# JuliaControl/ModelPredictiveControl.jl

Hardware: AMD Instinct MI355X
Metric: QP solves/sec (moveinput!) (higher is better)
Workload: dtype f64

## Files before the change

### modelpredictivecontrol.jl_amd/csrc/mpcqp_bodies.h

```cpp
#pragma once
#include <math.h>

#include <type_traits>

#include "mpcqp_types.h"

#if defined(MPCQP_PROFILE) && defined(__HIP_DEVICE_COMPILE__)
#define MPCQP_TIC() const long long tic_ = clock64()
#define MPCQP_TOC(i) prof_[i] += (double)(clock64() - tic_)
#define MPCQP_TICK(name) const long long name = clock64()
#define MPCQP_TOCK(i, name) prof_[i] += (double)(clock64() - name)
#elif defined(MPCQP_ISA_MARKERS) && defined(__HIP_DEVICE_COMPILE__)
#define MPCQP_MARK_(txt) do { __builtin_amdgcn_sched_barrier(0); asm volatile("; MPCQP_MARK " txt ::: "memory"); __builtin_amdgcn_sched_barrier(0); } while (0)
#define MPCQP_TIC() MPCQP_MARK_("tic")
#define MPCQP_TOC(i) MPCQP_MARK_("toc " #i)
#define MPCQP_TICK(name) MPCQP_MARK_("tic " #name)
#define MPCQP_TOCK(i, name) MPCQP_MARK_("toc " #i)
#define MPCQP_MTIC() MPCQP_MARK_("tic")
#define MPCQP_MTOC(name) MPCQP_MARK_("toc " name)
#else
#define MPCQP_TIC() ((void)0)
#define MPCQP_TOC(i) ((void)0)
#define MPCQP_TICK(name) ((void)0)
#define MPCQP_TOCK(i, name) ((void)0)
// ... 152 lines not shown
    }
    static bool matches(const Dims& d) { return matches_dims(d) && d.gmask == GMASK; }
};

template <class DM>
constexpr bool has_w() {
    if constexpr (DM::is_static) return DM::nw > 0;
    else return true;
}

constexpr int NROWARR = 7;

struct Carve {
    int S, Phi, zero, z, dz, q, zlo, zhi, gt, rd, dinv, zb, xh, F, tA[NPAIR], tB[NPAIR], ucum, exT, Wm;
    int rows[NROWARR];
    int jl, blk;
    int total;
};

template <class DM>
MPCQP_HD constexpr bool one_row_per_lane() {
    if constexpr (DM::is_static) return DM::nZ <= WAVE;
    else return false;
}

template <class DM>
MPCQP_HD constexpr int hwq_() {
    if constexpr (DM::is_static) {
        constexpr int n = (DM::nY + WAVE - 1) / WAVE;
        return (DM::nZ <= WAVE && n <= 4) ? n : 0;
    } else {
        return 0;
    }
}

template <class DM>
MPCQP_HD inline int stride_S(const DM& d) {
    if constexpr (DM::is_static) return DM::sp;
    else return d.ny * d.nu;
}

template <class DM>
MPCQP_HD inline int zpad_S(const DM&) {
    if constexpr (DM::is_static) return DM::zpad;
    else return 0;
}
// ... 515 lines not shown
                acc1 += ok ? p1 : 0.0;
            }
            if constexpr (REG) mine_k += scale * (acc0 + acc1);
            else out[k] += scale * (acc0 + acc1);
        }
    }

    MPCQP_HD static void unpack_idx(int idx, int& i, int& ip) {
        i = (int)((sqrt(8.0 * idx + 1.0) - 1.0) * 0.5);
        while (i * (i + 1) / 2 > idx) --i;
        while ((i + 1) * (i + 2) / 2 <= idx) ++i;
        ip = idx - i * (i + 1) / 2;
    }

#if defined(__HIP_DEVICE_COMPILE__)
    typedef double v4d __attribute__((ext_vector_type(4)));
    template <int I0, int NT, class F>
    static __device__ __forceinline__ void etde_passes(F& f) {
        if constexpr (I0 < NT) {
            f(std::integral_constant<int, I0>{});
            etde_passes<(I0 == 0 ? 2 : I0 + 1), NT>(f);
        }
    }
    __device__ __forceinline__ int EtDE_add_mfma(const double* dd, double* P, double scale, const double* tb,
                                                 const double* Hg = nullptr, bool ow = false) {
        if constexpr (W::NTEAM > 1) { static_assert(W::WV == 0, MPCQP_POST_WV0); w.post(TJ_ETDE, (int)(dd - sm), (int)(P - sm), tb ? (int)(tb - sm) : 0, (ow ? 1 : 0) | (Hg ? 2 : 0) | (tb ? 4 : 0), scale); }
        const int e = EtDE_share(dd, P, scale, tb ? tb : dd, Hg, ow, tb != nullptr);
        if constexpr (W::NTEAM > 1) w.join();
        return e;
    }
    __device__ __forceinline__ int EtDE_share(const double* dd, double* P, double scale, const double* tb, const double* Hg, bool ow, bool has_tb) {
        return EtDE_share_(dd, P, scale, tb, Hg, ow, has_tb);
    }
    __device__ __forceinline__ int EtDE_share_(const double* dd, double* P, double scale, const double* tb, const double* Hg, bool ow, bool has_tb) {
        ow = ow || Hg != nullptr;
        constexpr int NU = DM::nu, NY = DM::ny, NDU = DM::nDU, NYR = DM::nY, SP = DM::sp, RS = DM::rs;
        constexpr int NT = (NDU + 15) / 16, NK = (NYR + 3) / 4;
        const int li = w.lane & 15, lk = w.lane >> 4;
        const int lkp = (NY % 4 == 0) ? (((lk & 1) << 1) | (lk >> 1)) : lk;
        int offI[NT], offL[NT], jI[NT];
        MPCQP_UNROLL
        for (int I = 0; I < NT; ++I) {
            const int i = 16 * I + li;
            const int j = i / NU, cc = i - j * NU;
            const int tj = jl(i < NDU ? j : 0);
            jI[I] = i < NDU ? tj : (1 << 20);
            offI[I] = -tj * SP + cc;
            offL[I] = offI[I] + lkp * RS;
        }
        constexpr int IE = NDU / 16, LE = NDU % 16;
        int eps_t0 = -1;
        if (DM::neps && has_tb && IE < NT) {
            int v = (jl((16 * IE) / NU) * NY) / 4;
            v = v < NK ? v : NK;
            if ((4 * v) % NY != 0) v = 0;
            eps_t0 = (4 * v) / NY;
        }
// ... 10 lines not shown
        }
        auto pass = [&](auto I0c) {
            constexpr int I0 = decltype(I0c)::value;
            if constexpr (W::NTEAM > 1) {
                if constexpr (!team_mine_mfma<W>(I0 == 0 ? 0 : I0 - 1)) return;
            }
            constexpr int MAXT = NT + 1;
            constexpr int I1 = (I0 == 0 && NT > 1) ? 1 : I0;
            v4d acc[2][MAXT];
            MPCQP_UNROLL
            for (int x = 0; x < 2; ++x) {
                MPCQP_UNROLL
                for (int J = 0; J < MAXT; ++J) acc[x][J] = v4d{0.0, 0.0, 0.0, 0.0};
            }
            const bool erow = DM::neps && has_tb && IE >= I0 && IE <= I1;
            auto entry_ok = [&](int I, int J, int reg) {
                const bool eI = erow && I == IE;
                const int il = 4 * reg + lk;
                const bool rowok = 16 * I + 15 < NDU || 16 * I + il < NDU;
                const bool colok = 16 * J + 15 < NDU || 16 * J + li < NDU;
                const bool low = J < I || li <= il;
                return colok && ((rowok && low) || (eI && il == LE));
            };
            auto entry_idx = [&](int I, int J, int reg) {
                const int G = 4 * I + reg;
                return 8 * G * (G + 1) + 16 * J + 4 * (G + 1) * lk + li;
            };
            double hreg[2][MAXT][4];
            auto hload = [&]() {
                MPCQP_UNROLL
                for (int I = I0; I <= I1; ++I) {
                    MPCQP_UNROLL
                    for (int J = 0; J <= I; ++J) {
                        MPCQP_UNROLL
                        for (int reg = 0; reg < 4; ++reg)
                            hreg[I - I0][J][reg] = Hg[entry_ok(I, J, reg) ? (unsigned)entry_idx(I, J, reg) : 0u];
                    }
                }
            };
            constexpr bool LATEH = !VREG && NT > 4;
            if (Hg && !VREG && !LATEH) hload();
            auto kfirst = [&](int I) {
                int v = (jl((16 * I) / NU) * NY) / 4;
                v = v < NK ? v : NK;
                if (erow && I == IE) { if ((4 * v) % NY != 0) v = 0; }
                return v;
            };
            const int kB = (I1 > I0) ? kfirst(I1) : NK;
            const int kA = kfirst(I0) < kB ? kfirst(I0) : kB;
            const int zoff = (int)((sm + c.zero) - S);
            struct Ops { double dv, tbv, e[NT]; };
            auto kload = [&](int kk, Ops& o) {
                o.tbv = 0.0;
                if constexpr (NY % 4 == 0) {
                    const int t = (4 * kk) / NY, a0 = 4 * kk - t * NY;
                    const int base = t * SP + a0 * RS;
                    o.dv = dd[4 * kk + lkp];
                    if (erow) o.tbv = tb[4 * kk + lkp];
                    MPCQP_UNROLL
// ... 71 lines not shown
            for (int kk = kA; kk < kB1; ++kk) {
                if (PIPE) { kload(kk + 1, nxt); MPCQP_SCHED_FENCE(); kcomp(cur, true, false); MPCQP_SCHED_FENCE(); cur = nxt; }
                else { kload(kk, cur); kcomp(cur, true, false); }
            }
            if (LATEH && I1 == I0) {
                if (Hg) hload();
                MPCQP_SCHED_FENCE();
                MPCQP_PRAGMA(unroll MPCQP_ETDE_UNROLL)
                for (int kk = kB1; kk < kB; ++kk) {
                    if (PIPE) { kload(kk + 1, nxt); MPCQP_SCHED_FENCE(); kcomp(cur, true, false); MPCQP_SCHED_FENCE(); cur = nxt; }
                    else { kload(kk, cur); kcomp(cur, true, false); }
                }
            }
            if (I1 > I0) {
                if (LATEH && Hg) hload();
                MPCQP_PRAGMA(unroll MPCQP_ETDE_UNROLL)
                for (int kk = kB; kk < NK; ++kk) {
                    if (PIPE) { kload(kk + 1, nxt); MPCQP_SCHED_FENCE(); kcomp(cur, true, true); MPCQP_SCHED_FENCE(); cur = nxt; }
                    else { kload(kk, cur); kcomp(cur, true, true); }
                }
            }
            }
            if (Hg && VREG) hload();
            if (ow) {
                MPCQP_UNROLL
                for (int I = I0; I <= I1; ++I) {
                    MPCQP_UNROLL
                    for (int J = 0; J <= I; ++J) {
                        MPCQP_UNROLL
                        for (int reg = 0; reg < 4; ++reg)
                            if (entry_ok(I, J, reg))
                                P[entry_idx(I, J, reg)] = Hg ? fma(scale, acc[I - I0][J][reg], hreg[I - I0][J][reg]) : scale * acc[I - I0][J][reg];
                    }
                }
                return;
            }
            double* const trash = sm + c.zero + 4;
            MPCQP_UNROLL
            for (int I = I0; I <= I1; ++I) {
                MPCQP_UNROLL
                for (int J = 0; J <= I; ++J) {
                    double* pp_[4];
                    double old_[4];
                    MPCQP_UNROLL
                    for (int reg = 0; reg < 4; ++reg) {
                        pp_[reg] = entry_ok(I, J, reg) ? P + entry_idx(I, J, reg) : trash;
                        old_[reg] = *pp_[reg];
                    }
                    MPCQP_UNROLL
                    for (int reg = 0; reg < 4; ++reg) *pp_[reg] = fma(scale, acc[I - I0][J][reg], old_[reg]);
                }
            }
        };
        etde_passes<0, NT>(pass);
        if constexpr (DM::neps != 0 && W::WV == 0) {
            if (ow && !Hg) {
                if constexpr (IE >= NT) {
                    for (int k = w.lane; k < NDU; k += WAVE) P[pk(NDU, k)] = 0.0;
                }
                if (w.lane == 0) P[pk(NDU, NDU)] = 0.0;
            } else if (Hg) {
                if constexpr (IE >= NT) {
                    for (int k = w.lane; k < NDU; k += WAVE) P[pk(NDU, k)] = Hg[pk(NDU, k)];
                }
                if (w.lane == 0) P[pk(NDU, NDU)] = Hg[pk(NDU, NDU)];
            }
        }
        return eps_t0;
    }
#endif

    MPCQP_HD int EtDE_add(const double* dd, double* P, double scale = 1.0, const double* tb = nullptr,
                          const double* Hg = nullptr, bool ow = false) {
#if defined(__HIP_DEVICE_COMPILE__)
        if constexpr (DM::is_static) return EtDE_add_mfma(dd, P, scale, tb, Hg, ow);
#endif
        const int ny = d.ny, nu = d.nu, nDU = d.nDU;
        const int nstrip = pk_size(nDU) / 4;
        for (int st = w.lane; st < nstrip; st += WAVE) {
            int g = (int)((sqrt(1.0 + 2.0 * st) - 1.0) * 0.5);
            while (2 * g * (g + 1) > st) --g;
            while (2 * (g + 1) * (g + 2) <= st) ++g;
            const int rem = st - 2 * g * (g + 1);
            const int i = 4 * g + rem / (g + 1), ip0 = 4 * (rem % (g + 1));
            if (i >= nDU) continue;
            const int j = i / nu, cc = i - j * nu, t0 = jl(j);
            const double* S2[4];
            MPCQP_UNROLL
            for (int u = 0; u < 4; ++u) {
                const int ip = ip0 + u <= i ? ip0 + u : i;
                const int j2 = ip / nu, c2 = ip - j2 * nu;
                S2[u] = S + (t0 - jl(j2)) * sp + c2;
            }
            const double* S1 = S + cc;
            const double* dt = dd + t0 * ny;
            double acc[4] = {0.0, 0.0, 0.0, 0.0};
            for (int t = t0; t < d.Hp; ++t) {
                for (int a = 0; a < ny; ++a) {
// ... 433 lines not shown
    RowStore<DM> rows;
    double *z, *dz, *q, *zlo, *zhi, *gt, *rd, *F, *Phi;
    int mact;
    double wsum;
    double nh;
    double delta;
    double prof_[16] = {0};
    double myinvd = 0.0;
    double myd_ = 0.0;
    bool chol_broke = false;
    bool fold_H = false;
    bool h_Lnz = false;
    double h2n_ = 0.0, h2l_ = 0.0;
    static constexpr int HWQ = hwq_<DM>();
    double hwy_[HWQ > 0 ? HWQ : 1] = {0.0};
    MPCQP_HD static constexpr bool hwy_cached() { return hwq_<DM>() > 0; }
    MPCQP_HD double hwy(int k) const {
        double v = hwy_[0];
        MPCQP_UNROLL
        for (int q_ = 1; q_ < HWQ; ++q_) v = (k >= WAVE * q_) ? hwy_[q_] : v;
        return v;
    }

    MPCQP_HD Step(Qp<W, DM>& qp_)
        : qp(qp_), w(qp_.w), d(qp_.d), m(qp_.m), b(qp_.b), sm(qp_.sm), c(qp_.c),
          rows(qp_.d, qp_.sm, qp_.c, qp_.w.lane) {
        z = sm + c.z; dz = sm + c.dz; q = sm + c.q; zlo = sm + c.zlo; zhi = sm + c.zhi;
        gt = sm + c.gt; rd = sm + c.rd; F = sm + c.F;
        Phi = qp.Phi;
        delta = d.dual_reg;
    }

    MPCQP_HD double stepc_at(int a, int k) const { return m.stepc[((size_t)b * SC_N + a) * d.nDU + k]; }

    MPCQP_HD double soft_init(int g, int k) const {
        if (!d.neps) return 0.0;
        const double* p = nullptr;
        double def = 0.0;
        switch (g) {
            case 2 * P_U: p = m.C_umin; break;
            case 2 * P_U + 1: p = m.C_umax; break;
            case 2 * P_DU: p = m.C_dumin; break;
            case 2 * P_DU + 1: p = m.C_dumax; break;
            case 2 * P_Y: p = m.C_ymin; def = 1.0; break;
            case 2 * P_Y + 1: p = m.C_ymax; def = 1.0; break;
            case 2 * P_X: p = m.c_x0min; def = 1.0; break;
// ... 596 lines not shown
        qp.Et_apply_add(tY, rd, 2.0);
        double suf = 0.0;
        if (h_Lnz && d.nDU <= WAVE) {
            const double pre = qp.block_prefix(w.lane < d.nDU ? z[w.lane] : 0.0);
            suf = qp.block_suffix(w.lane < d.nDU ? H2L(w.lane) * pre : 0.0);
        }
        for (int k = w.lane; k < d.nZ; k += WAVE) {
            const double hn = one_row_per_lane<DM>() ? h2n_ : H2N_load(k);
            rd[k] = (k < d.nDU ? rd[k] + suf : 0.0) + hn * z[k];
        }
        w.sync();
        MPCQP_TOC(2);
    }

    MPCQP_HD void load_H() {
        if constexpr (W::NTEAM > 1) { static_assert(W::WV == 0, MPCQP_POST_WV0); w.post(TJ_LOADH); }
        load_H_share();
        if constexpr (W::NTEAM > 1) w.join();
        w.sync();
    }
    MPCQP_HD void load_H_share() {
        const double* H = m.Hpk + (size_t)b * d.npk;
        constexpr int NB = 8;
        const int n = d.npk, stride = WAVE * W::NTEAM;
        for (int i0 = WAVE * W::WV; i0 < n; i0 += NB * stride) {
            double v[NB];
            MPCQP_UNROLL
            for (int q_ = 0; q_ < NB; ++q_) { const int i = i0 + w.lane + stride * q_; v[q_] = H[i < n ? i : 0]; }
            MPCQP_UNROLL
            for (int q_ = 0; q_ < NB; ++q_) { const int i = i0 + w.lane + stride * q_; if (i < n) Phi[i] = v[q_]; }
        }
    }

    MPCQP_HD bool phi_direct() const {
#if defined(__HIP_DEVICE_COMPILE__)
        return fold_H || (DM::is_static && qp.pair_on(P_Y));
#else
        return fold_H;
#endif
    }
    MPCQP_HD bool etde_overwrites() const {
#if defined(__HIP_DEVICE_COMPILE__)
        return DM::is_static && qp.pair_on(P_Y);
#else
        return false;
#endif
    }

    MPCQP_HD void GtDG_urows_share() {
        const int nu = d.nu, nDU = d.nDU;
        const double* tU = sm + c.tA[P_U];
        for (int k = w.lane + WAVE * ((W::WV + W::NTEAM - 1) % W::NTEAM); k < nDU; k += WAVE * W::NTEAM) {
            const int j = k / nu, cc = k - j * nu;
            const double suf = tU[k];
            MPCQP_PRAGMA(unroll MPCQP_URMW_UNROLL)
            for (int j2 = 0; j2 <= j; ++j2) Phi[pk(k, j2 * nu + cc)] += suf;
        }
    }
    MPCQP_HD void GtDG_xrows_share() {
        const int nDU = d.nDU, ntri = nDU * (nDU + 1) / 2;
        const double* tX = sm + c.tA[P_X];
        for (int idx = w.lane + WAVE * W::WV; idx < ntri; idx += WAVE * W::NTEAM) {
            int i, ip;
            Qp<W, DM>::unpack_idx(idx, i, ip);
            double acc = 0.0;
            for (int r = 0; r < d.nxh; ++r) acc += qp.Xat(r, i) * tX[r] * qp.Xat(r, ip);
            Phi[pk(i, ip)] += acc;
        }
    }
    MPCQP_HD void GtDG_wrows_share() {
        if constexpr (has_w<DM>()) {
            const int nu = d.nu, nDU = d.nDU, ntri = nDU * (nDU + 1) / 2, nw = d.nw;
            const double* dW = sm + c.tA[P_W];
            for (int idx = w.lane + WAVE * W::WV; idx < ntri; idx += WAVE * W::NTEAM) {
                int i, ip;
                Qp<W, DM>::unpack_idx(idx, i, ip);
                const int j = i / nu, cc = i - j * nu, j2 = ip / nu, c2 = ip - j2 * nu;
                double acc = 0.0;
                for (int t = 0; t <= d.Hp; ++t)
                    for (int iw = 0; iw < nw; ++iw) {
                        const double dk = dW[t * nw + iw];
                        if (dk != 0.0) acc += dk * qp.Ew_at(t, iw, j, cc) * qp.Ew_at(t, iw, j2, c2);
                    }
                Phi[pk(i, ip)] += acc;
            }
        }
    }

    template <class Fn>
    MPCQP_HD void add_GtDG(Fn dd) {
        MPCQP_TIC();
        const int nu = d.nu, nDU = d.nDU, nZ = d.nZ;
        double ee = 0.0;
        for_pairs([&](int p, int k, Row* r0, Row* r1) {
            double dmin = 0.0, dmax = 0.0, cmin = 0.0, cmax = 0.0;
            if (r0 && fin(*r0)) { dmin = dd(*r0); cmin = r0->cs; }
            if (r1 && fin(*r1)) { dmax = dd(*r1); cmax = r1->cs; }
            double hw = 0.0;
            if (fold_H) {
                if (p == P_Y) hw = hwy_cached() ? hwy(k) : (k < d.nY ? 2.0 * m.Mdiag[(size_t)b * d.nY + k] : 0.0);
                else if (p == P_U) hw = H2L(k);
            }
            sm[c.tA[p] + k] = dmin + dmax + hw;
            if (p != P_BOX) {
                sm[c.tB[p] + k] = cmin * dmin - cmax * dmax;
                ee += cmin * cmin * dmin + cmax * cmax * dmax;
            }
        });
        ee = w.sum(ee);
        w.sync();
        if (fold_H && !etde_overwrites()) {
            for (int i = w.lane; i < d.npk; i += WAVE) Phi[i] = 0.0;
            w.sync();
        }
        bool epsY = qp.pair_on(P_Y), epsU = qp.pair_on(P_U);
        if constexpr (has_w<DM>()) {
            if (qp.pair_on(P_W) && d.neps) {
                qp.W_fold(sm + c.tB[P_W], sm + c.tB[P_Y], !epsY, sm + c.tB[P_U], !epsU);
                epsY = epsU = true;
            }
        }
        MPCQP_TOC(3);
        int eps_t0 = -1;
        if (qp.pair_on(P_Y)) {
            MPCQP_TIC();
            eps_t0 = qp.EtDE_add(sm + c.tA[P_Y], Phi, 1.0, d.neps ? sm + c.tB[P_Y] : nullptr,
                                 (phi_direct() && !fold_H) ? m.Hpk + (size_t)b * d.npk : nullptr, fold_H && etde_overwrites());
            w.sync();
            MPCQP_TOC(4);
        }
        MPCQP_TICK(tic5_);
        if (qp.pair_on(P_U) && nDU <= WAVE) {
            const double* tU = sm + c.tA[P_U];
            const int k = w.lane < nDU ? w.lane : 0;
            const int j = k / nu, cc = k - j * nu;
            const double suf = qp.block_suffix(w.lane < nDU ? tU[k] : 0.0);
            double* const trash = sm + c.zero + 4;
            double* const row = Phi + pk(k, cc);
            if constexpr (DM::is_static) {
                double* q_[DM::Hc];
                double old_[DM::Hc];
                MPCQP_UNROLL
                for (int j2 = 0; j2 < DM::Hc; ++j2) {
                    q_[j2] = (j2 <= j && w.lane < nDU) ? row + j2 * nu : trash;
                    old_[j2] = *q_[j2];
                }
                MPCQP_UNROLL
                for (int j2 = 0; j2 < DM::Hc; ++j2) *q_[j2] = old_[j2] + suf;
            } else {
                for (int j2 = 0; j2 < d.Hc; ++j2) {
                    double* const q_ = (j2 <= j && w.lane < nDU) ? row + j2 * nu : trash;
                    *q_ += suf;
                }
            }
        } else if (qp.pair_on(P_U)) {
            double* tU = sm + c.tA[P_U];
            w.sync();
            block_scan(tU, tU, true);
            if constexpr (W::NTEAM > 1) { static_assert(W::WV == 0, MPCQP_POST_WV0); w.post(TJ_UROWS); }
            GtDG_urows_share();
            if constexpr (W::NTEAM > 1) w.join();
        }
        if (qp.pair_on(P_X)) {
            w.sync();
            if constexpr (W::NTEAM > 1) { static_assert(W::WV == 0, MPCQP_POST_WV0); w.post(TJ_XROWS); }
            GtDG_xrows_share();
            if constexpr (W::NTEAM > 1) w.join();
        }
        if constexpr (has_w<DM>()) {
            if (qp.pair_on(P_W)) {
                w.sync();
                if constexpr (W::NTEAM > 1) { static_assert(W::WV == 0, MPCQP_POST_WV0); w.post(TJ_WROWS); }
                GtDG_wrows_share();
                if constexpr (W::NTEAM > 1) w.join();
            }
        }
        w.sync();
        for (int k = w.lane; k < nZ; k += WAVE) {
            double acc = 0.0;
            if (qp.pair_on(P_BOX)) acc += sm[c.tA[P_BOX] + k];
            if (k < nDU && qp.pair_on(P_DU)) acc += sm[c.tA[P_DU] + k];
            if (k == nZ - 1 && d.neps) acc += ee;
            if (fold_H) acc += one_row_per_lane<DM>() ? h2n_ : H2N_load(k);
            Phi[pk(k, k)] += acc;
        }
        if (d.neps) {
            double* st = dz;
            double sufB = 0.0;
            if (epsU && nDU <= WAVE) sufB = qp.block_suffix(w.lane < nDU ? sm[c.tB[P_U] + w.lane] : 0.0);
            for (int k = w.lane; k < nDU; k += WAVE) {
                double acc = 0.0;
                if (qp.pair_on(P_DU)) acc += sm[c.tB[P_DU] + k];
                if (epsU && nDU <= WAVE) acc += sufB;
                else if (epsU) {
                    const int j = k / nu, cc = k - j * nu;
                    const double* tU = sm + c.tB[P_U];
                    MPCQP_UNROLL4
                    for (int jj = j; jj < d.Hc; ++jj) acc += tU[jj * nu + cc];
                }
                if (qp.pair_on(P_X)) {
                    const double* tX = sm + c.tB[P_X];
                    for (int i = 0; i < d.nxh; ++i) acc += qp.Xat(i, k) * tX[i];
                }
                st[k] = acc;
            }
            if (epsY && eps_t0 != 0) qp.Et_apply_add(sm + c.tB[P_Y], st, 1.0, eps_t0);
            for (int k = w.lane; k < nDU; k += WAVE) Phi[pk(nZ - 1, k)] += st[k];
        }
        w.sync();
        MPCQP_TOCK(5, tic5_);
    }

    MPCQP_HD static long long clock64_() {
#if defined(MPCQP_PROFILE) && defined(__HIP_DEVICE_COMPILE__)
        return clock64();
#else
        return 0;
#endif
    }

    MPCQP_HD static void load4(const double* p, double* x) {
#if defined(__HIP_DEVICE_COMPILE__)
        typedef double v2d_ __attribute__((ext_vector_type(2)));
        const v2d_ a = reinterpret_cast<const v2d_*>(p)[0], b2 = reinterpret_cast<const v2d_*>(p)[1];
        x[0] = a.x; x[1] = a.y; x[2] = b2.x; x[3] = b2.y;
#else
        x[0] = p[0]; x[1] = p[1]; x[2] = p[2]; x[3] = p[3];
#endif
    }
    MPCQP_HD static void store4(double* p, const double* x) {
// ... 5 lines not shown
        p[0] = x[0]; p[1] = x[1]; p[2] = x[2]; p[3] = x[3];
#endif
    }

#if defined(__HIP_DEVICE_COMPILE__)
    template <int P>
    __device__ __forceinline__ void chol_panel_update() {
        if constexpr (W::NTEAM > 1) { static_assert(W::WV == 0, MPCQP_POST_WV0); w.post(TJ_PANEL, P); }
        chol_panel_share<P>();
        if constexpr (W::NTEAM > 1) w.join();
    }
    template <int P>
    __device__ __forceinline__ void chol_panel_share() {
        typedef double v4d_ __attribute__((ext_vector_type(4)));
        constexpr int n = DM::nZ, NT = (n + 15) / 16;
        if constexpr (P < NT) {
            const int li = w.lane & 15, lk = w.lane >> 4;
            auto mine = [](int I) { return team_mine_mfma<W>(I - P); };
            const double* X[NT];
            v4d_ acc[NT];
            MPCQP_UNROLL
            for (int I = P; I < NT; ++I) {
                const int row = 16 * I + li < n ? 16 * I + li : n - 1;
                X[I] = Phi + pk(row, 0) + lk;
                acc[I] = v4d_{0.0, 0.0, 0.0, 0.0};
            }
            if constexpr (team_any_mfma<W>(NT - P)) {
            MPCQP_PRAGMA(unroll MPCQP_PANEL_UNROLL)
            for (int kk = 0; kk < 4 * P; ++kk) {
                const double bb = X[P][4 * kk];
                const double bs = one_row_per_lane<DM>() ? bb * gt[4 * kk + lk] : bb;
                if (mine(P)) acc[P] = __builtin_amdgcn_mfma_f64_16x16x4f64(bb, bs, acc[P], 0, 0, 0);
                MPCQP_UNROLL
                for (int I = P + 1; I < NT; ++I)
                    if (mine(I)) acc[I] = __builtin_amdgcn_mfma_f64_16x16x4f64(X[I][4 * kk], bs, acc[I], 0, 0, 0);
            }
            }
            double* const trash = sm + c.zero + 4;
            MPCQP_UNROLL
            for (int I = P; I < NT; ++I) {
                if (!mine(I)) continue;
                double* pp_[4];
                double old_[4];
                MPCQP_UNROLL
                for (int reg = 0; reg < 4; ++reg) {
                    const int row = 16 * I + lk + 4 * reg, col = 16 * P + li;
                    pp_[reg] = (row < n && col <= row) ? Phi + pk(row, col) : trash;
                    old_[reg] = *pp_[reg];
                }
                MPCQP_UNROLL
                for (int reg = 0; reg < 4; ++reg) *pp_[reg] = old_[reg] - acc[I][reg];
            }
            w.sync();
        }
    }
#endif

#if defined(__HIP_DEVICE_COMPILE__)
    template <int P>
    __device__ __forceinline__ void panel_dispatch(int p) {
        if constexpr (P < (DM::nZ + 15) / 16) {
            if (p == P) chol_panel_share<P>();
            else panel_dispatch<P + 1>(p);
        }
    }
#endif

#if defined(__HIP_DEVICE_COMPILE__)
    template <int P, int Bk>
    __device__ __forceinline__ void chol_block_update() {
        typedef double v4d_ __attribute__((ext_vector_type(4)));
        constexpr int n = DM::nZ, NT = (n + 15) / 16, K0 = 16 * P + 4 * Bk;
        const int li = w.lane & 15, lk = w.lane >> 4;
        double x[NT];
        MPCQP_UNROLL
        for (int T = P; T < NT; ++T) {
            const int row = 16 * T + li < n ? 16 * T + li : n - 1;
            x[T] = Phi[pk(row, 0) + K0 + lk];
        }
        const double xPs = one_row_per_lane<DM>() ? x[P] * gt[K0 + lk] : x[P];
        double* const trash = sm + c.zero + 4;
        double* q_[NT][4];
        double old_[NT][4];
        MPCQP_UNROLL
        for (int T = P; T < NT; ++T) {
            MPCQP_UNROLL
            for (int r = Bk + 1; r < 4; ++r) {
                if (16 * P + 4 * r >= n) continue;
                const int row = 16 * T + li, col = 16 * P + 4 * r + lk;
                q_[T][r] = (row < n && col <= row) ? Phi + pk(row, col) : trash;
                old_[T][r] = *q_[T][r];
            }
        }
        MPCQP_UNROLL
        for (int T = P; T < NT; ++T) {
            const v4d_ acc = __builtin_amdgcn_mfma_f64_16x16x4f64(xPs, x[T], v4d_{0.0, 0.0, 0.0, 0.0}, 0, 0, 0);
            MPCQP_UNROLL
            for (int r = Bk + 1; r < 4; ++r) {
                if (16 * P + 4 * r >= n) continue;
                *q_[T][r] = old_[T][r] - acc[r];
            }
        }
        w.sync();
    }

    template <int K0>
    __device__ __forceinline__ void chol_static(double thr) {
        constexpr int n = DM::nZ, CB = 4, P = K0 / 16, Bk = (K0 % 16) / 4;
        const int i = w.lane;
        const bool act = i < n;
        const int rowi = pk(act ? i : 0, 0);
        if constexpr (Bk == 0 && P > 0) chol_panel_update<P>();
        const bool mine = act && i >= K0;
        double v[CB], lk[CB];
        load4(mine ? Phi + rowi + K0 : sm + c.zero, v);
        constexpr int NCL = (n - K0 < CB) ? n - K0 : CB;
        MPCQP_UNROLL
        for (int cc = 0; cc < CB; ++cc) {
            if (cc < NCL) {
                const int k = K0 + cc;
                const double nidb = -w.bcast(rcp(v[cc]), k);
                lk[cc] = v[cc] * nidb;
                MPCQP_UNROLL
                for (int c2 = cc + 1; c2 < NCL; ++c2) v[c2] = fma(v[cc], w.bcast(lk[cc], K0 + c2), v[c2]);
            } else {
                lk[cc] = 0.0;
            }
        }
        if (mine) {
            const double t0 = (i & 1) ? v[1] : v[0], t1 = (i & 1) ? v[3] : v[2];
            myd_ = (i & 2) ? t1 : t0;
            gt[i] = myd_;
            MPCQP_UNROLL
            for (int cc = 0; cc < CB; ++cc) lk[cc] = (i > K0 + cc) ? lk[cc] : 0.0;
            store4(Phi + rowi + K0, lk);
        }
        w.sync();
        if constexpr (K0 + CB < n) {
            if constexpr (Bk < 3) chol_block_update<P, Bk>();
            chol_static<K0 + CB>(thr);
        }
    }
#endif

    MPCQP_HD void cholesky() {
        if (d.nZ > WAVE) { cholesky_big(); return; }
        cholesky_();
    }
    MPCQP_HD void cholesky_() {
        MPCQP_TIC();
        const int n = d.nZ;
        const int i = w.lane;
        const bool act = i < n;
        const int rowi = pk(act ? i : 0, 0);
        const double dia = act ? Phi[rowi + i] : 1.0;
        const double thr = 1e-14 * fabs(dia);
        const double* zero4 = sm + c.zero;
        myinvd = 0.0;
        constexpr int CB = 4;
#if defined(__HIP_DEVICE_COMPILE__)
        if constexpr (one_row_per_lane<DM>()) {
            chol_static<0>(thr);
            chol_broke = w.any(act && !(myd_ > thr));
            myinvd = act ? rcp(myd_) : 0.0;
            w.sync();
            MPCQP_TOC(6);
            return;
        }
#endif
        MPCQP_NOUNROLL
        for (int k0 = 0; k0 < n; k0 += CB) {
            const bool mine = act && i >= k0;
            double v[CB];
            load4(mine ? Phi + rowi + k0 : zero4, v);
            if (mine && k0 > 0) {
                const double* Li = Phi + rowi;
                const int rb = pk(k0, 0), rs = k0 + CB;
                const double* Lk[CB];
// ... 27 lines not shown
            }
            w.sync();
        }
        myinvd = fmx(myinvd, 1e-32);
        chol_broke = w.any(act && myinvd <= 1e-32);
        MPCQP_TOC(6);
    }

    MPCQP_HD static double rsqrt_(double x) {
#if defined(__HIP_DEVICE_COMPILE__)
        const double r = __builtin_amdgcn_rsq(x);
        return r * fma(-0.5 * x * r, r, 1.5);
#else
        return 1.0 / sqrt(x);
#endif
    }

#if defined(__HIP_DEVICE_COMPILE__)
    template <int T>
    __device__ __forceinline__ void solve_fwd_load(double (*cf)[4], const int rowi, const bool act) {
        constexpr int n = DM::nZ, K0 = 16 * T, KT = (n - K0 < 16) ? n - K0 : 16, NC = (KT + 3) / 4;
        const int i = w.lane;
        MPCQP_UNROLL
        for (int u = 0; u < NC; ++u) load4((act && i >= K0 + 4 * u) ? Phi + rowi + K0 + 4 * u : sm + c.zero, cf[u]);
    }
    template <int T>
    __device__ __forceinline__ void solve_bwd_load(double (*cb)[4]) {
        constexpr int n = DM::nZ, K0 = 16 * T, KT = (n - K0 < 16) ? n - K0 : 16, NC = (KT + 3) / 4;
        const int i = w.lane;
        MPCQP_UNROLL
        for (int u = 0; u < NC; ++u) {
            const int k0 = K0 + 4 * u;
            const double* p = solve_zero_region() ? ((i < k0 + 4 && i < n) ? Phi + pk(k0, 0) + i : sm + c.S)
                                                  : Phi + pk(k0, 0) + (i < k0 + 4 ? i : 0);
            MPCQP_UNROLL
            for (int e = 0; e < 4; ++e) cb[u][e] = (k0 + e < n) ? p[e * (k0 + 4)] : 0.0;
        }
    }
    template <int T>
    __device__ __forceinline__ void solve_fwd_tile(double& r, double (*cf)[4], const int rowi, const bool act) {
        constexpr int n = DM::nZ, NT = (n + 15) / 16, K0 = 16 * T, KT = (n - K0 < 16) ? n - K0 : 16, NC = (KT + 3) / 4;
        double nx[4][4];
        if constexpr (T + 1 < NT) solve_fwd_load<T + 1>(nx, rowi, act);
        else solve_bwd_load<NT - 1>(nx);
        MPCQP_SCHED_FENCE();
        MPCQP_UNROLL
        for (int u = 0; u < NC; ++u) chain_sw<1 << T, false>(u, r, cf[u]);
        if constexpr (T + 1 < NT) {
            const double y = w.fetch(r, K0 + (w.lane & 15));
            double a0 = 0.0, a1 = 0.0;
            MPCQP_UNROLL
            for (int u = 0; u < NC; ++u) rows_sw<0xf & ~((2 << T) - 1)>(u, (u & 1) ? a1 : a0, y, cf[u]);
            r += a0 + a1;
            MPCQP_SCHED_FENCE();
            solve_fwd_tile<T + 1>(r, nx, rowi, act);
// ... 26 lines not shown
            for (int u = 0; u < NC; ++u) rows_sw<(1 << T) - 1>(u, (u & 1) ? a1 : a0, x, cb[u]);
            r += a0 + a1;
            solve_bwd_tile<T - 1>(r, nx, act);
        }
    }
    template <int ROWS, bool REV>
    __device__ __forceinline__ void chain_sw(int u, double& r, const double* cc) {
        switch (u) {
            case 0: W::template chain4<0, ROWS, REV>(r, cc[0], cc[1], cc[2], cc[3]); break;
            case 1: W::template chain4<4, ROWS, REV>(r, cc[0], cc[1], cc[2], cc[3]); break;
            case 2: W::template chain4<8, ROWS, REV>(r, cc[0], cc[1], cc[2], cc[3]); break;
            default: W::template chain4<12, ROWS, REV>(r, cc[0], cc[1], cc[2], cc[3]); break;
        }
    }
    template <int ROWS>
    __device__ __forceinline__ void rows_sw(int u, double& a, double x, const double* cc) {
        switch (u) {
            case 0: W::template fmabc4<0, ROWS>(a, x, cc[0], cc[1], cc[2], cc[3]); break;
            case 1: W::template fmabc4<4, ROWS>(a, x, cc[0], cc[1], cc[2], cc[3]); break;
            case 2: W::template fmabc4<8, ROWS>(a, x, cc[0], cc[1], cc[2], cc[3]); break;
            default: W::template fmabc4<12, ROWS>(a, x, cc[0], cc[1], cc[2], cc[3]); break;
        }
    }
    static constexpr bool solve_zero_region() { return DM::zpad * DM::sp >= 3 * (DM::nZ + 3) + 4; }
    __device__ __forceinline__ void solve_static() {
        const int i = w.lane;
        solve_static_reg(i < DM::nZ ? gt[i] : 0.0);
    }
    __device__ __forceinline__ double solve_static_reg(double r) {
        constexpr int n = DM::nZ;
        const int i = w.lane;
        const bool act = i < n;
        const int rowi = pk(act ? i : 0, 0);
        double cf[4][4];
        solve_fwd_load<0>(cf, rowi, act);
        solve_fwd_tile<0>(r, cf, rowi, act);
        if (act) dz[i] = r;
        w.sync();
        return act ? r : 0.0;
    }
#endif

    MPCQP_HD void solve_into_dz() {
        w.relane();
        if (d.nZ > WAVE) { solve_big(); return; }
        MPCQP_TIC();
#if defined(__HIP_DEVICE_COMPILE__)
        if constexpr (one_row_per_lane<DM>()) {
            solve_static();
            MPCQP_TOC(7);
            return;
        }
#endif
        const int n = d.nZ;
        const int i = w.lane;
        const bool act = i < n;
// ... 406 lines not shown
            int j = 0;
            MPCQP_PRAGMA(unroll MPCQP_HZ_UNROLL)
            for (; j + 1 <= k; j += 2) { h0 += Hk[j] * z[j]; h1 += Hk[j + 1] * z[j + 1]; }
            if (j <= k) h0 += Hk[j] * z[j];
            MPCQP_PRAGMA(unroll MPCQP_HZ_UNROLL)
            for (int jj = k + 1; jj < n; ++jj) h1 += Hp_[pk(jj, k)] * z[jj];
            rd[k] = h0 + h1;
        }
    }
    MPCQP_HD void dual_residual(const double* Hp_, double& rdn, double& nd_) {
        const int n = d.nZ;
        double mx = 0.0, sc = 0.0;
        if constexpr (W::NTEAM > 1) {
            if (Hp_) {
                static_assert(W::WV == 0, MPCQP_POST_WV0); w.post(TJ_HZ, Hp_ == Phi ? 1 : 0);
                if (Hp_ == Phi) Hz_rows_share(Phi);
                else Hz_rows_share(m.Hpk + (size_t)b * d.npk);
                w.join();
                Hp_ = nullptr;
            }
        }
        for (int k = w.lane; k < n; k += WAVE) {
            double h0 = 0.0, h1 = 0.0;
            if (Hp_) {
                const double* Hk = Hp_ + pk(k, 0);
                int j = 0;
                MPCQP_PRAGMA(unroll MPCQP_HZ_UNROLL)
                for (; j + 1 <= k; j += 2) { h0 += Hk[j] * z[j]; h1 += Hk[j + 1] * z[j + 1]; }
                if (j <= k) h0 += Hk[j] * z[j];
                MPCQP_PRAGMA(unroll MPCQP_HZ_UNROLL)
                for (int jj = k + 1; jj < n; ++jj) h1 += Hp_[pk(jj, k)] * z[jj];
            } else {
                h0 = rd[k];
            }
            const double hz = h0 + h1;
            const double r = hz + q[k] + gt[k];
            rd[k] = r;
            mx = fmx_abs(mx, r);
            sc = fmx_abs(fmx_abs(fmx_abs(sc, q[k]), hz), gt[k]);
        }
        rdn = w.maxv(mx);
        nd_ = 1.0 + w.maxv(sc);
        w.sync();
    }

    MPCQP_HD void residuals(double& mu, double& rpn, double& rdn, double& nd_, bool gz_kept = false) {
        const int n = d.nZ;
// ... 587 lines not shown
```

### modelpredictivecontrol.jl_amd/csrc/mpcqp_types.h

```cpp
#pragma once
#include <stdint.h>

#if defined(__HIPCC__)
#define MPCQP_HD __host__ __device__ __attribute__((always_inline))
#define MPCQP_UNROLL _Pragma("unroll")
#define MPCQP_UNROLL4 _Pragma("unroll 4")
#define MPCQP_NOUNROLL _Pragma("nounroll")
#if defined(__HIP_DEVICE_COMPILE__)
#define MPCQP_SCHED_FENCE() __builtin_amdgcn_sched_barrier(0)
#else
#define MPCQP_SCHED_FENCE() ((void)0)
#endif
#else
#define MPCQP_SCHED_FENCE() ((void)0)
#define MPCQP_HD
#define MPCQP_UNROLL
#define MPCQP_UNROLL4
#define MPCQP_NOUNROLL
#endif

#define MPCQP_KERNEL_REV 15

namespace mpcqp {

enum TeamJob { TJ_EXIT = 0, TJ_ETDE = 1, TJ_PANEL = 2, TJ_EV = 3, TJ_ETW = 4, TJ_UROWS = 5, TJ_WROWS = 6, TJ_XROWS = 7, TJ_PANELROWS = 8, TJ_LOADH = 9, TJ_HZ = 10 };
#define MPCQP_POST_WV0 "only wavefront 0 of a team posts jobs: a helper that reached this call would wait at the barrier for ever"


enum { P_BOX = 0, P_U = 1, P_DU = 2, P_Y = 3, P_X = 4, P_W = 5, NPAIR = 6, NGROUP = 12 };

constexpr int WAVE = 64;
constexpr double BIG = 1e300;

MPCQP_HD constexpr int eps_host_group(uint32_t gmask, int neps) {
    return !neps ? -1 : ((gmask >> (2 * P_Y + 1)) & 1u) ? 2 * P_Y + 1 : ((gmask >> (2 * P_Y)) & 1u) ? 2 * P_Y : -1;
}

struct Dims {
    int B, nxh, nu, ny, nd, Hp, Hc, neps;
    int nZ, nDU, nU, nY, nD;
    int nw, nW;
    int npk;
    uint32_t gmask;
    int rowoff_[NGROUP + 1];
// ... 45 lines not shown
    int nym;
};

struct StepIO {
    const double *xhat0, *lastu0, *Ry, *Ru, *d0, *Dhat0;
    double *Z, *u0, *Yhat0;
    int32_t *status, *iters;
    double *q_keep, *F_keep;
    const double* lam_prev;
    double* lam_out;
    double *prof;
    double *audit;
    const double* kf_K;
    const int* kf_iym;
    const double* kf_y0m;
    double* xhat0_out;
    int kf_nym, kf_predict;
    int kf_late;
};

MPCQP_HD constexpr int pk(int i, int j) { return 4 * ((i >> 2) + 1) * (2 * (i >> 2) + (i & 3)) + j; }
MPCQP_HD constexpr int pk_size(int n) { return pk(n, 0); }

}
```

Baseline: 4.761 million.

## Store Phi in column-block-major layout for single-team static kernels

Result: faster. 4.877 million (median of 6 runs) (+2.4%).

```diff
diff --git a/modelpredictivecontrol.jl_amd/csrc/mpcqp_bodies.h b/modelpredictivecontrol.jl_amd/csrc/mpcqp_bodies.h
--- a/modelpredictivecontrol.jl_amd/csrc/mpcqp_bodies.h
+++ b/modelpredictivecontrol.jl_amd/csrc/mpcqp_bodies.h
@@ -198,6 +198,21 @@
 MPCQP_HD constexpr bool one_row_per_lane() {
     if constexpr (DM::is_static) return DM::nZ <= WAVE;
     else return false;
+}
+
+template <class W, class DM>
+MPCQP_HD constexpr bool phi_layout() {
+#if defined(__HIP_DEVICE_COMPILE__)
+    if constexpr (DM::is_static) return DM::nZ <= WAVE && W::NTEAM == 1;
+    else return false;
+#else
+    return false;
+#endif
+}
+template <class W, class DM>
+MPCQP_HD constexpr int phi_ix(int i, int j) {
+    if constexpr (phi_layout<W, DM>()) return phi(DM::nZ, i, j);
+    else return pk(i, j);
 }
 
 template <class DM>
@@ -759,17 +774,21 @@
             etde_passes<(I0 == 0 ? 2 : I0 + 1), NT>(f);
         }
     }
+    template <bool PH = false>
     __device__ __forceinline__ int EtDE_add_mfma(const double* dd, double* P, double scale, const double* tb,
                                                  const double* Hg = nullptr, bool ow = false) {
         if constexpr (W::NTEAM > 1) { static_assert(W::WV == 0, MPCQP_POST_WV0); w.post(TJ_ETDE, (int)(dd - sm), (int)(P - sm), tb ? (int)(tb - sm) : 0, (ow ? 1 : 0) | (Hg ? 2 : 0) | (tb ? 4 : 0), scale); }
-        const int e = EtDE_share(dd, P, scale, tb ? tb : dd, Hg, ow, tb != nullptr);
+        const int e = EtDE_share<PH>(dd, P, scale, tb ? tb : dd, Hg, ow, tb != nullptr);
         if constexpr (W::NTEAM > 1) w.join();
         return e;
     }
+    template <bool PH = false>
     __device__ __forceinline__ int EtDE_share(const double* dd, double* P, double scale, const double* tb, const double* Hg, bool ow, bool has_tb) {
-        return EtDE_share_(dd, P, scale, tb, Hg, ow, has_tb);
-    }
+        return EtDE_share_<PH>(dd, P, scale, tb, Hg, ow, has_tb);
+    }
+    template <bool PH>
     __device__ __forceinline__ int EtDE_share_(const double* dd, double* P, double scale, const double* tb, const double* Hg, bool ow, bool has_tb) {
+        static_assert(!PH || phi_layout<W, DM>(), "column-block-major Phi outside its kernels");
         ow = ow || Hg != nullptr;
         constexpr int NU = DM::nu, NY = DM::ny, NDU = DM::nDU, NYR = DM::nY, SP = DM::sp, RS = DM::rs;
         constexpr int NT = (NDU + 15) / 16, NK = (NYR + 3) / 4;
@@ -826,9 +845,22 @@
                 const bool low = J < I || li <= il;
                 return colok && ((rowok && low) || (eI && il == LE));
             };
-            auto entry_idx = [&](int I, int J, int reg) {
+            auto entry_idx_pk = [&](int I, int J, int reg) {
                 const int G = 4 * I + reg;
                 return 8 * G * (G + 1) + 16 * J + 4 * (G + 1) * lk + li;
+            };
+            int eb[MAXT];
+            auto entry_base = [&]() {
+                if constexpr (PH) {
+                    const int q_ = li >> 2;
+                    const int eb0 = 4 * q_ * (DM::nZ - 2 - 2 * q_) + (li & 3) + 4 * lk;
+                    MPCQP_UNROLL
+                    for (int J = 0; J <= I1; ++J) eb[J] = eb0 + 16 * J * (DM::nZ - 2 - 8 * J) - 64 * J * q_;
+                }
+            };
+            auto entry_idx = [&](int I, int J, int reg) {
+                if constexpr (PH) return eb[J] + 64 * I + 16 * reg;
+                else return entry_idx_pk(I, J, reg);
             };
             double hreg[2][MAXT][4];
             auto hload = [&]() {
@@ -838,7 +870,7 @@
                     for (int J = 0; J <= I; ++J) {
                         MPCQP_UNROLL
                         for (int reg = 0; reg < 4; ++reg)
-                            hreg[I - I0][J][reg] = Hg[entry_ok(I, J, reg) ? (unsigned)entry_idx(I, J, reg) : 0u];
+                            hreg[I - I0][J][reg] = Hg[entry_ok(I, J, reg) ? (unsigned)entry_idx_pk(I, J, reg) : 0u];
                     }
                 }
             };
@@ -956,6 +988,7 @@
             }
             }
             if (Hg && VREG) hload();
+            entry_base();
             if (ow) {
                 MPCQP_UNROLL
                 for (int I = I0; I <= I1; ++I) {
@@ -987,27 +1020,29 @@
             }
         };
         etde_passes<0, NT>(pass);
+        auto pix = [](int i, int j) { if constexpr (PH) return phi(DM::nZ, i, j); else return pk(i, j); };
         if constexpr (DM::neps != 0 && W::WV == 0) {
             if (ow && !Hg) {
                 if constexpr (IE >= NT) {
-                    for (int k = w.lane; k < NDU; k += WAVE) P[pk(NDU, k)] = 0.0;
-                }
-                if (w.lane == 0) P[pk(NDU, NDU)] = 0.0;
+                    for (int k = w.lane; k < NDU; k += WAVE) P[pix(NDU, k)] = 0.0;
+                }
+                if (w.lane == 0) P[pix(NDU, NDU)] = 0.0;
             } else if (Hg) {
                 if constexpr (IE >= NT) {
-                    for (int k = w.lane; k < NDU; k += WAVE) P[pk(NDU, k)] = Hg[pk(NDU, k)];
-                }
-                if (w.lane == 0) P[pk(NDU, NDU)] = Hg[pk(NDU, NDU)];
+                    for (int k = w.lane; k < NDU; k += WAVE) P[pix(NDU, k)] = Hg[pk(NDU, k)];
+                }
+                if (w.lane == 0) P[pix(NDU, NDU)] = Hg[pk(NDU, NDU)];
             }
         }
         return eps_t0;
     }
 #endif
 
+    template <bool PH = false>
     MPCQP_HD int EtDE_add(const double* dd, double* P, double scale = 1.0, const double* tb = nullptr,
                           const double* Hg = nullptr, bool ow = false) {
 #if defined(__HIP_DEVICE_COMPILE__)
-        if constexpr (DM::is_static) return EtDE_add_mfma(dd, P, scale, tb, Hg, ow);
+        if constexpr (DM::is_static) return EtDE_add_mfma<PH>(dd, P, scale, tb, Hg, ow);
 #endif
         const int ny = d.ny, nu = d.nu, nDU = d.nDU;
         const int nstrip = pk_size(nDU) / 4;
@@ -1487,6 +1522,11 @@
         return v;
     }
 
+    static constexpr bool PHL = phi_layout<W, DM>();
+    MPCQP_HD static constexpr int ix(int i, int j) { return phi_ix<W, DM>(i, j); }
+    MPCQP_HD static constexpr int rowoff(int i) { if constexpr (PHL) return 4 * i; else return pk(i, 0); }
+    MPCQP_HD static constexpr int coloff(int j) { if constexpr (PHL) return phi_col(DM::nZ, j); else return j; }
+
     MPCQP_HD Step(Qp<W, DM>& qp_)
         : qp(qp_), w(qp_.w), d(qp_.d), m(qp_.m), b(qp_.b), sm(qp_.sm), c(qp_.c),
           rows(qp_.d, qp_.sm, qp_.c, qp_.w.lane) {
@@ -2129,6 +2169,24 @@
     MPCQP_HD void load_H_share() {
         const double* H = m.Hpk + (size_t)b * d.npk;
         constexpr int NB = 8;
+        if constexpr (PHL) {
+            constexpr int n_ = DM::nZ, G_ = (n_ + 3) / 4, NPK = pk_size(n_);
+            for (int i0 = 0; i0 < NPK; i0 += NB * WAVE) {
+                double v[NB];
+                MPCQP_UNROLL
+                for (int q_ = 0; q_ < NB; ++q_) {
+                    const int s_ = i0 + w.lane + WAVE * q_, ss = s_ < NPK ? s_ : 0;
+                    int cb = 0;
+                    MPCQP_UNROLL
+                    for (int c2 = 1; c2 < G_; ++c2) cb += (ss >= phi_blk(n_, c2)) ? 1 : 0;
+                    const int o = ss - phi_blk(n_, cb);
+                    v[q_] = H[pk(4 * cb + (o >> 2), 4 * cb + (o & 3))];
+                }
+                MPCQP_UNROLL
+                for (int q_ = 0; q_ < NB; ++q_) { const int s_ = i0 + w.lane + WAVE * q_; if (s_ < NPK) Phi[s_] = v[q_]; }
+            }
+            return;
+        }
         const int n = d.npk, stride = WAVE * W::NTEAM;
         for (int i0 = WAVE * W::WV; i0 < n; i0 += NB * stride) {
             double v[NB];
@@ -2161,7 +2219,7 @@
             const int j = k / nu, cc = k - j * nu;
             const double suf = tU[k];
             MPCQP_PRAGMA(unroll MPCQP_URMW_UNROLL)
-            for (int j2 = 0; j2 <= j; ++j2) Phi[pk(k, j2 * nu + cc)] += suf;
+            for (int j2 = 0; j2 <= j; ++j2) Phi[ix(k, j2 * nu + cc)] += suf;
         }
     }
     MPCQP_HD void GtDG_xrows_share() {
@@ -2172,7 +2230,7 @@
             Qp<W, DM>::unpack_idx(idx, i, ip);
             double acc = 0.0;
             for (int r = 0; r < d.nxh; ++r) acc += qp.Xat(r, i) * tX[r] * qp.Xat(r, ip);
-            Phi[pk(i, ip)] += acc;
+            Phi[ix(i, ip)] += acc;
         }
     }
     MPCQP_HD void GtDG_wrows_share() {
@@ -2189,7 +2247,7 @@
                         const double dk = dW[t * nw + iw];
                         if (dk != 0.0) acc += dk * qp.Ew_at(t, iw, j, cc) * qp.Ew_at(t, iw, j2, c2);
                     }
-                Phi[pk(i, ip)] += acc;
+                Phi[ix(i, ip)] += acc;
             }
         }
     }
@@ -2231,7 +2289,7 @@
         int eps_t0 = -1;
         if (qp.pair_on(P_Y)) {
             MPCQP_TIC();
-            eps_t0 = qp.EtDE_add(sm + c.tA[P_Y], Phi, 1.0, d.neps ? sm + c.tB[P_Y] : nullptr,
+            eps_t0 = qp.template EtDE_add<PHL>(sm + c.tA[P_Y], Phi, 1.0, d.neps ? sm + c.tB[P_Y] : nullptr,
                                  (phi_direct() && !fold_H) ? m.Hpk + (size_t)b * d.npk : nullptr, fold_H && etde_overwrites());
             w.sync();
             MPCQP_TOC(4);
@@ -2243,20 +2301,28 @@
             const int j = k / nu, cc = k - j * nu;
             const double suf = qp.block_suffix(w.lane < nDU ? tU[k] : 0.0);
             double* const trash = sm + c.zero + 4;
-            double* const row = Phi + pk(k, cc);
+            double* const row = Phi + (PHL ? 0 : pk(k, cc));
+            auto urow = [&](int j2) -> double* {
+                if constexpr (PHL) {
+                    if constexpr (DM::nu == 4) return Phi + 4 * k + cc + phi_col(DM::nZ, 4 * j2);
+                    else return Phi + ix(k, j2 * nu + cc);
+                } else {
+                    return row + j2 * nu;
+                }
+            };
             if constexpr (DM::is_static) {
                 double* q_[DM::Hc];
                 double old_[DM::Hc];
                 MPCQP_UNROLL
                 for (int j2 = 0; j2 < DM::Hc; ++j2) {
-                    q_[j2] = (j2 <= j && w.lane < nDU) ? row + j2 * nu : trash;
+                    q_[j2] = (j2 <= j && w.lane < nDU) ? urow(j2) : trash;
                     old_[j2] = *q_[j2];
                 }
                 MPCQP_UNROLL
                 for (int j2 = 0; j2 < DM::Hc; ++j2) *q_[j2] = old_[j2] + suf;
             } else {
                 for (int j2 = 0; j2 < d.Hc; ++j2) {
-                    double* const q_ = (j2 <= j && w.lane < nDU) ? row + j2 * nu : trash;
+                    double* const q_ = (j2 <= j && w.lane < nDU) ? urow(j2) : trash;
                     *q_ += suf;
                 }
             }
@@ -2289,7 +2355,7 @@
             if (k < nDU && qp.pair_on(P_DU)) acc += sm[c.tA[P_DU] + k];
             if (k == nZ - 1 && d.neps) acc += ee;
             if (fold_H) acc += one_row_per_lane<DM>() ? h2n_ : H2N_load(k);
-            Phi[pk(k, k)] += acc;
+            Phi[ix(k, k)] += acc;
         }
         if (d.neps) {
             double* st = dz;
@@ -2312,7 +2378,7 @@
                 st[k] = acc;
             }
             if (epsY && eps_t0 != 0) qp.Et_apply_add(sm + c.tB[P_Y], st, 1.0, eps_t0);
-            for (int k = w.lane; k < nDU; k += WAVE) Phi[pk(nZ - 1, k)] += st[k];
+            for (int k = w.lane; k < nDU; k += WAVE) Phi[ix(nZ - 1, k)] += st[k];
         }
         w.sync();
         MPCQP_TOCK(5, tic5_);
@@ -2364,21 +2430,29 @@
             MPCQP_UNROLL
             for (int I = P; I < NT; ++I) {
                 const int row = 16 * I + li < n ? 16 * I + li : n - 1;
-                X[I] = Phi + pk(row, 0) + lk;
+                if constexpr (!PHL) X[I] = Phi + pk(row, 0) + lk;
                 acc[I] = v4d_{0.0, 0.0, 0.0, 0.0};
             }
+            const double* const xb = Phi + 4 * li + lk;
+            const int lrow = 16 * (NT - 1) + li < n ? 16 * (NT - 1) + li : n - 1;
+            const double* const xl = (n % 16 == 0) ? xb : Phi + 4 * lrow + lk - 64 * (NT - 1);
+            auto Xop = [&](int I, int kk) -> double {
+                if constexpr (PHL) return (I == NT - 1 ? xl : xb)[coloff(4 * kk) + 64 * I];
+                else return X[I][4 * kk];
+            };
             if constexpr (team_any_mfma<W>(NT - P)) {
             MPCQP_PRAGMA(unroll MPCQP_PANEL_UNROLL)
             for (int kk = 0; kk < 4 * P; ++kk) {
-                const double bb = X[P][4 * kk];
+                const double bb = Xop(P, kk);
                 const double bs = one_row_per_lane<DM>() ? bb * gt[4 * kk + lk] : bb;
                 if (mine(P)) acc[P] = __builtin_amdgcn_mfma_f64_16x16x4f64(bb, bs, acc[P], 0, 0, 0);
                 MPCQP_UNROLL
                 for (int I = P + 1; I < NT; ++I)
-                    if (mine(I)) acc[I] = __builtin_amdgcn_mfma_f64_16x16x4f64(X[I][4 * kk], bs, acc[I], 0, 0, 0);
+                    if (mine(I)) acc[I] = __builtin_amdgcn_mfma_f64_16x16x4f64(Xop(I, kk), bs, acc[I], 0, 0, 0);
             }
             }
             double* const trash = sm + c.zero + 4;
+            double* const wb = Phi + (PHL ? phi_col(n, 16 * P + li) + 4 * lk : 0);
             MPCQP_UNROLL
             for (int I = P; I < NT; ++I) {
                 if (!mine(I)) continue;
@@ -2387,7 +2461,12 @@
                 MPCQP_UNROLL
                 for (int reg = 0; reg < 4; ++reg) {
                     const int row = 16 * I + lk + 4 * reg, col = 16 * P + li;
-                    pp_[reg] = (row < n && col <= row) ? Phi + pk(row, col) : trash;
+                    if constexpr (PHL) {
+                        const bool ok = (16 * I + 15 < n || row < n) && (I > P || col <= row);
+                        pp_[reg] = ok ? wb + 64 * I + 16 * reg : trash;
+                    } else {
+                        pp_[reg] = (row < n && col <= row) ? Phi + pk(row, col) : trash;
+                    }
                     old_[reg] = *pp_[reg];
                 }
                 MPCQP_UNROLL
@@ -2415,10 +2494,17 @@
         constexpr int n = DM::nZ, NT = (n + 15) / 16, K0 = 16 * P + 4 * Bk;
         const int li = w.lane & 15, lk = w.lane >> 4;
         double x[NT];
+        double* const xb = Phi + 4 * li + lk;
+        const int lrow = 16 * (NT - 1) + li < n ? 16 * (NT - 1) + li : n - 1;
+        const double* const xl = (n % 16 == 0) ? xb : Phi + 4 * lrow + lk - 64 * (NT - 1);
         MPCQP_UNROLL
         for (int T = P; T < NT; ++T) {
-            const int row = 16 * T + li < n ? 16 * T + li : n - 1;
-            x[T] = Phi[pk(row, 0) + K0 + lk];
+            if constexpr (PHL) {
+                x[T] = (T == NT - 1 ? xl : xb)[coloff(K0) + 64 * T];
+            } else {
+                const int row = 16 * T + li < n ? 16 * T + li : n - 1;
+                x[T] = Phi[pk(row, 0) + K0 + lk];
+            }
         }
         const double xPs = one_row_per_lane<DM>() ? x[P] * gt[K0 + lk] : x[P];
         double* const trash = sm + c.zero + 4;
@@ -2430,7 +2516,12 @@
             for (int r = Bk + 1; r < 4; ++r) {
                 if (16 * P + 4 * r >= n) continue;
                 const int row = 16 * T + li, col = 16 * P + 4 * r + lk;
-                q_[T][r] = (row < n && col <= row) ? Phi + pk(row, col) : trash;
+                if constexpr (PHL) {
+                    const bool ok = (16 * T + 15 < n || row < n) && (T > P || col <= row);
+                    q_[T][r] = ok ? xb + coloff(16 * P + 4 * r) + 64 * T : trash;
+                } else {
+                    q_[T][r] = (row < n && col <= row) ? Phi + pk(row, col) : trash;
+                }
                 old_[T][r] = *q_[T][r];
             }
         }
@@ -2451,11 +2542,12 @@
         constexpr int n = DM::nZ, CB = 4, P = K0 / 16, Bk = (K0 % 16) / 4;
         const int i = w.lane;
         const bool act = i < n;
-        const int rowi = pk(act ? i : 0, 0);
+        const int rowi = rowoff(act ? i : 0);
         if constexpr (Bk == 0 && P > 0) chol_panel_update<P>();
         const bool mine = act && i >= K0;
         double v[CB], lk[CB];
-        load4(mine ? Phi + rowi + K0 : sm + c.zero, v);
+        if constexpr (PHL) load4(Phi + rowi + coloff(K0), v);
+        else load4(mine ? Phi + rowi + K0 : sm + c.zero, v);
         constexpr int NCL = (n - K0 < CB) ? n - K0 : CB;
         MPCQP_UNROLL
         for (int cc = 0; cc < CB; ++cc) {
@@ -2475,7 +2567,7 @@
             gt[i] = myd_;
             MPCQP_UNROLL
             for (int cc = 0; cc < CB; ++cc) lk[cc] = (i > K0 + cc) ? lk[cc] : 0.0;
-            store4(Phi + rowi + K0, lk);
+            store4(Phi + rowi + coloff(K0), lk);
         }
         w.sync();
         if constexpr (K0 + CB < n) {
@@ -2495,7 +2587,7 @@
         const int i = w.lane;
         const bool act = i < n;
         const int rowi = pk(act ? i : 0, 0);
-        const double dia = act ? Phi[rowi + i] : 1.0;
+        const double dia = act ? Phi[PHL ? ix(i, i) : rowi + i] : 1.0;
         const double thr = 1e-14 * fabs(dia);
         const double* zero4 = sm + c.zero;
         myinvd = 0.0;
@@ -2569,7 +2661,7 @@
         constexpr int n = DM::nZ, K0 = 16 * T, KT = (n - K0 < 16) ? n - K0 : 16, NC = (KT + 3) / 4;
         const int i = w.lane;
         MPCQP_UNROLL
-        for (int u = 0; u < NC; ++u) load4((act && i >= K0 + 4 * u) ? Phi + rowi + K0 + 4 * u : sm + c.zero, cf[u]);
+        for (int u = 0; u < NC; ++u) load4((act && i >= K0 + 4 * u) ? Phi + rowi + coloff(K0 + 4 * u) : sm + c.zero, cf[u]);
     }
     template <int T>
     __device__ __forceinline__ void solve_bwd_load(double (*cb)[4]) {
@@ -2578,6 +2670,14 @@
         MPCQP_UNROLL
         for (int u = 0; u < NC; ++u) {
             const int k0 = K0 + 4 * u;
+            if constexpr (PHL) {
+                const int cbase = phi_col(n, (i < n) ? i : 0);
+                const double* p = solve_zero_region() ? ((i < k0 + 4 && i < n) ? Phi + cbase + 4 * k0 : sm + c.S)
+                                                      : Phi + (i < k0 + 4 ? cbase : 0) + 4 * k0;
+                MPCQP_UNROLL
+                for (int e = 0; e < 4; ++e) cb[u][e] = (k0 + e < n) ? p[4 * e] : 0.0;
+                continue;
+            }
             const double* p = solve_zero_region() ? ((i < k0 + 4 && i < n) ? Phi + pk(k0, 0) + i : sm + c.S)
                                                   : Phi + pk(k0, 0) + (i < k0 + 4 ? i : 0);
             MPCQP_UNROLL
@@ -2650,7 +2750,7 @@
             default: W::template fmabc4<12, ROWS>(a, x, cc[0], cc[1], cc[2], cc[3]); break;
         }
     }
-    static constexpr bool solve_zero_region() { return DM::zpad * DM::sp >= 3 * (DM::nZ + 3) + 4; }
+    static constexpr bool solve_zero_region() { return DM::zpad * DM::sp >= (PHL ? 13 : 3 * (DM::nZ + 3) + 4); }
     __device__ __forceinline__ void solve_static() {
         const int i = w.lane;
         solve_static_reg(i < DM::nZ ? gt[i] : 0.0);
@@ -2659,7 +2759,7 @@
         constexpr int n = DM::nZ;
         const int i = w.lane;
         const bool act = i < n;
-        const int rowi = pk(act ? i : 0, 0);
+        const int rowi = rowoff(act ? i : 0);
         double cf[4][4];
         solve_fwd_load<0>(cf, rowi, act);
         solve_fwd_tile<0>(r, cf, rowi, act);
@@ -3112,7 +3212,15 @@
         }
         for (int k = w.lane; k < n; k += WAVE) {
             double h0 = 0.0, h1 = 0.0;
-            if (Hp_) {
+            if (PHL && Hp_ == Phi) {
+                int j = 0;
+                MPCQP_PRAGMA(unroll MPCQP_HZ_UNROLL)
+                for (; j + 1 <= k; j += 2) { h0 += Phi[ix(k, j)] * z[j]; h1 += Phi[ix(k, j + 1)] * z[j + 1]; }
+                if (j <= k) h0 += Phi[ix(k, j)] * z[j];
+                const double* const Hc = Phi + coloff(k);
+                MPCQP_PRAGMA(unroll MPCQP_HZ_UNROLL)
+                for (int jj = k + 1; jj < n; ++jj) h1 += Hc[4 * jj] * z[jj];
+            } else if (Hp_) {
                 const double* Hk = Hp_ + pk(k, 0);
                 int j = 0;
                 MPCQP_PRAGMA(unroll MPCQP_HZ_UNROLL)
diff --git a/modelpredictivecontrol.jl_amd/csrc/mpcqp_types.h b/modelpredictivecontrol.jl_amd/csrc/mpcqp_types.h
--- a/modelpredictivecontrol.jl_amd/csrc/mpcqp_types.h
+++ b/modelpredictivecontrol.jl_amd/csrc/mpcqp_types.h
@@ -19,7 +19,7 @@
 #define MPCQP_NOUNROLL
 #endif
 
-#define MPCQP_KERNEL_REV 15
+#define MPCQP_KERNEL_REV 16
 
 namespace mpcqp {
 
@@ -111,4 +111,34 @@
 MPCQP_HD constexpr int pk(int i, int j) { return 4 * ((i >> 2) + 1) * (2 * (i >> 2) + (i & 3)) + j; }
 MPCQP_HD constexpr int pk_size(int n) { return pk(n, 0); }
 
+MPCQP_HD constexpr int phi_blk(int n, int c) { return 4 * c * n - 8 * c * (c - 1); }
+MPCQP_HD constexpr int phi_col(int n, int j) { return 4 * (j >> 2) * (n - 2 * (j >> 2) - 2) + (j & 3); }
+MPCQP_HD constexpr int phi(int n, int i, int j) { return phi_col(n, j) + 4 * i; }
+constexpr bool phi_bijective(int n) {
+    const int G = (n + 3) / 4, size = pk_size(n);
+    if (phi_blk(n, G) != size) return false;
+    bool seen[pk_size(64)] = {};
+    int cnt = 0;
+    for (int c = 0; c < G; ++c) {
+        if (phi_col(n, 4 * c) < 0 || phi_col(n, 4 * c) != phi_blk(n, c) - 16 * c) return false;
+        for (int i = 4 * c; i < n; ++i)
+            for (int j = 4 * c; j < 4 * c + 4; ++j) {
+                const int s = phi(n, i, j);
+                if (s < 0 || s >= size || seen[s]) return false;
+                if (s != phi_blk(n, c) + 4 * (i - 4 * c) + (j & 3)) return false;
+                seen[s] = true;
+                ++cnt;
+            }
+    }
+    return cnt == size;
 }
+template <int N>
+struct PhiProof {
+    static_assert(phi_bijective(N), "phi(n, i, j) is not a bijection onto [0, pk_size(n))");
+    static constexpr bool ok = PhiProof<N - 1>::ok;
+};
+template <>
+struct PhiProof<0> { static constexpr bool ok = true; };
+static_assert(PhiProof<64>::ok, "column-block-major layout of Phi, n = 1 .. 64");
+
+}
```
